# zhangxiaochen95/uav_bs_ctrl

Measured on AMD Instinct MI355X. Metric: env-steps/sec (MADRQN, 8 UBS x 80 GT), higher is better.
Workload: dtype f32

## Files before the change

### include/uavgnn.h

```cpp
#ifndef UAVGNN_H
#define UAVGNN_H

#include <stddef.h>
#include <stdint.h>

#ifdef __cplusplus
extern "C" {
#endif

#define UAVGNN_VERSION 101

#define UAVGNN_EINVAL (-1000)
#define UAVGNN_EUNSUPPORTED (-1001)
#define UAVGNN_EWORKSPACE (-1002)

typedef void* uavgnn_stream_t;

int uavgnn_version(void);

const char* uavgnn_strerror(int code);

int uavgnn_gatv2_fwd(const float* x_src, int E, int F_src, const float* x_dst, int F_dst, const int32_t* seg_off,
                     const int32_t* dst_order, int N, const float* W_s, const float* b_s, const float* W_d, const float* b_d, const float* attn,
                     const float* W_r, const float* b_r, int nh, int D, float slope, float* out, int ld_out,
// ... 205 lines not shown
int uavgnn_gru_cell_x3_supported(int K_in, int H);
long long uavgnn_gru_cell_x3_workspace_bytes(int K_in, int H);
int uavgnn_gru_split_weights(const float* W_ih, int K_in, const float* W_hh, int H, void* planes, uavgnn_stream_t stream);
int uavgnn_gru_cell_fwd_x3(const float* inp, int ld_inp, int K_in, const float* h, int N, int H, const void* planes,
                           const float* b_ih, const float* b_hh, float* h_out, float* pre_save, uavgnn_stream_t stream);
int uavgnn_gru_cell_fwd_x3_cat(const float* inp, int ld_inp, int K1, const float* inp2, int ld_inp2, int K2, const float* h,
                               int N, int H, const void* planes, const float* b_ih, const float* b_hh, float* h_out,
                               float* pre_save, uavgnn_stream_t stream);
#define UAVGNN_GRU_STAGING_BLOCKS 1
int uavgnn_gru_cell_fwd_x3_opts(const float* inp, int ld_inp, int K1, const float* inp2, int ld_inp2, int K2, const float* h,
                                int N, int H, const void* planes, const float* b_ih, const float* b_hh, float* h_out,
                                float* pre_save, int flags, uavgnn_stream_t stream);
int uavgnn_gru_cell_h2_supported(int K_in, int H);
long long uavgnn_gru_cell_h2_workspace_bytes(int K_in, int H);
int uavgnn_gru_split_weights_h2(const float* W_ih, int K_in, const float* W_hh, int H, void* planes, uavgnn_stream_t stream);
int uavgnn_gru_cell_fwd_h2(const float* inp, int ld_inp, int K1, const float* inp2, int ld_inp2, int K2, const float* h, int N, int H,
                           const float* row_absmax, const void* planes, const float* b_ih, const float* b_hh, float* h_out,
                           float* pre_save, uavgnn_stream_t stream);
int uavgnn_row_absmax(const float* a1, int ld1, int K1, const float* a2, int ld2, int K2, const float* a3, int ld3, int K3, int N,
                      float* out, uavgnn_stream_t stream);
int uavgnn_head_supported(int H, int A);
int uavgnn_head_fwd(const float* h, int ld_h, int N, int H, const float* W, int ld_w, const float* b, int A, float* q, int ld_q,
                    uavgnn_stream_t stream);
int uavgnn_head_duel_supported(int H, int A);
int uavgnn_head_fwd_duel(const float* h, int ld_h, int N, int H, const float* W_adv, int ld_w, const float* w_v, const float* b_adv,
                         const float* b_v, int A, float* q, int ld_q, uavgnn_stream_t stream);
int uavgnn_gru_rec_supported(int H);
int uavgnn_gru_rec_fwd(const float* gi, int ld_gi, const float* h, int ld_h, int N, int H, const float* W_hh, const float* b_hh,
                       float* h_out, int ld_ho, float* pre_save, uavgnn_stream_t stream);
int uavgnn_gru_rec_bwd(const float* pre, const float* h, int ld_h, const float* d_hout, const float* d_carry, int N, int H,
                       const float* W_hh, float* d_gi, float* d_gh, float* dh_prev, uavgnn_stream_t stream);
#define UAVGNN_GEMM_ACCUMULATE 1
#define UAVGNN_GEMM_RELU 2
#define UAVGNN_GEMM_STAGING_INTERLEAVED 4
#define UAVGNN_GEMM_TILE_128 8
#define UAVGNN_GEMM_TILE_64 16
int uavgnn_gemm_x3_supported(int M, int N, int K);
int uavgnn_split_bf16x3(const float* W, int ld, int R, int C, int transpose, void* planes, uavgnn_stream_t stream);
int uavgnn_gemm_nt_x3(const float* X, int ldx, int M, int K, const void* planes, int N, const float* bias, float* Y, int ldy,
                      int epilogue, uavgnn_stream_t stream);
int uavgnn_gemm_nt_x3_cat(const float* X, int ldx, int K1, const float* X2, int ldx2, int M, int K, const void* planes, int N,
                          const float* bias, float* Y, int ldy, int epilogue, uavgnn_stream_t stream);
int uavgnn_gemm_nt_x3_rowmax(const float* X, int ldx, int M, int K, const void* planes, int N, const float* bias, float* Y, int ldy,
                             int epilogue, float* rowmax_out, uavgnn_stream_t stream);

int uavgnn_gemm_tn_x3_chunks(long long n_rows, int Mo, int Ko);
int uavgnn_gemm_tn_x3(const float* dY, int ldy, int Mo, const float* X, int ldx, int Ko, long long n_rows, float* partials,
                      int S, int accumulate, uavgnn_stream_t stream);
int uavgnn_col_absmax(const float* x, long long ld, long long n, int C, float* out, uavgnn_stream_t stream);
int uavgnn_gemm_tn_h2_supported(long long n_rows, int Mo, int Ko);
int uavgnn_gemm_tn_h2_chunks(long long n_rows, int Mo, int Ko);
int uavgnn_gemm_tn_h2(const float* dY, long long ldy, int Mo, const float* X, long long ldx, int Ko, long long n_rows,
                      const float* colmax_y, const float* colmax_x, float* partials, int S, int accumulate, uavgnn_stream_t stream);
int uavgnn_gru_gates_bwd_fused(const float* pre, const float* h, const float* d_hout, int N, int H, float* d_gi, float* d_gh,
                               float* d_h, uavgnn_stream_t stream);
int uavgnn_gru_gates_bwd_fused_head(const float* pre, const float* h, const float* d_hout, const float* dq, int n_out,
                                    const float* W_out, int N, int H, float* d_gi, float* d_gh, float* d_h,
                                    uavgnn_stream_t stream);
int uavgnn_gru_gates_bwd_sum_rows(int N, int H);
int uavgnn_gru_gates_bwd_fused_sums(const float* pre, const float* h, const float* d_hout, const float* dq, int n_out,
                                    const float* W_out, int N, int H, float* d_gi, float* d_gh, float* d_h, float* col_sums,
                                    uavgnn_stream_t stream);

long long uavgnn_gru_cell_bwd_workspace_bytes(int K_in, int H);
int uavgnn_gru_split_weights_bwd(const float* W_ih, int K_in, const float* W_hh, int H, void* planes, uavgnn_stream_t stream);
int uavgnn_gru_cell_bwd(const float* pre, const float* h, const float* d_hout, int N, int K_in, int H, const void* planes_bwd,
                        float* d_gi, float* d_gh, float* d_inp, int ld_dinp, float* d_h, uavgnn_stream_t stream);

#define UAVGNN_WS_GATV2_BWD 1
#define UAVGNN_WS_DEGREE_ORDER 2
#define UAVGNN_WS_CSC_TRANSPOSE 3
#define UAVGNN_WS_GRU_PLANES 4
#define UAVGNN_WS_GRU_BWD_PLANES 5
#define UAVGNN_WS_GEMM_PLANES 6
#define UAVGNN_WS_GEMM_TN_PARTIALS 7
#define UAVGNN_WS_K1_IMAGE 8
long long uavgnn_workspace_bytes(int kind, long long a, long long b, long long c);

#ifdef __cplusplus
}
#endif
#endif
```

### uav_bs_ctrl_amd/_lib.py

```python
from __future__ import annotations

import ctypes
import os

import torch as th

_HERE = os.path.dirname(os.path.abspath(__file__))
LIB_PATH = os.environ.get("UAVGNN_LIB") or os.path.join(_HERE, "csrc", "libuavgnn.so")

_c_fp = ctypes.c_void_p
_c_ip = ctypes.c_void_p
_c_int = ctypes.c_int
_c_f32 = ctypes.c_float
_c_st = ctypes.c_void_p

SIGNATURES = {
    "uavgnn_version": (_c_int, []),
    "uavgnn_strerror": (ctypes.c_char_p, [_c_int]),
    "uavgnn_gatv2_fwd": (_c_int, [_c_fp, _c_int, _c_int, _c_fp, _c_int, _c_ip, _c_ip, _c_int, _c_fp, _c_fp, _c_fp, _c_fp, _c_fp,
                                  _c_fp, _c_fp, _c_int, _c_int, _c_f32, _c_fp, _c_int, _c_fp, _c_st]),
    "uavgnn_gatv2_fwd_valu": (_c_int, [_c_fp, _c_int, _c_int, _c_fp, _c_int, _c_ip, _c_ip, _c_int, _c_fp, _c_fp, _c_fp, _c_fp, _c_fp,
                                       _c_fp, _c_fp, _c_int, _c_int, _c_f32, _c_fp, _c_int, _c_fp, _c_st]),
    "uavgnn_gatv2_fwd_mfma": (_c_int, [_c_fp, _c_int, _c_int, _c_fp, _c_int, _c_ip, _c_ip, _c_int, _c_fp, _c_fp, _c_fp, _c_fp, _c_fp,
                                       _c_fp, _c_fp, _c_int, _c_int, _c_f32, _c_fp, _c_int, _c_fp, _c_st]),
# ... 38 lines not shown
    "uavgnn_talk_compact": (_c_int, [_c_fp, _c_int, _c_int, _c_f32, _c_ip, _c_ip, _c_ip, _c_ip, _c_st]),
    "uavgnn_build_graph_small_max_agents": (_c_int, []),
    "uavgnn_build_graph_small": (_c_int, [_c_fp, _c_int, _c_int, _c_fp, _c_int, _c_int, _c_fp, _c_int, _c_int, _c_f32, _c_ip, _c_ip,
                                          _c_ip, _c_fp, _c_fp, _c_ip, _c_ip, _c_ip, _c_st]),
    "uavgnn_degree_order_workspace_bytes": (ctypes.c_size_t, [_c_int]),
    "uavgnn_degree_order": (_c_int, [_c_ip, _c_int, _c_ip, ctypes.c_void_p, ctypes.c_size_t, _c_st]),
    "uavgnn_csc_transpose_workspace_bytes": (ctypes.c_size_t, [_c_int]),
    "uavgnn_csc_transpose": (_c_int, [_c_ip, _c_ip, _c_int, _c_int, _c_ip, _c_ip, _c_ip, ctypes.c_void_p,
                                      ctypes.c_size_t, _c_st]),
    "uavgnn_csc_transpose_env": (_c_int, [_c_ip, _c_ip, _c_ip, _c_int, _c_int, _c_ip, _c_ip, _c_ip, _c_st]),
    "uavgnn_talk_attn_env_supported": (_c_int, [_c_int, _c_int, _c_int]),
    "uavgnn_tarmac_msg_supported": (_c_int, [_c_int, _c_int, _c_int, _c_int]),
    "uavgnn_tarmac_msg_weight_bytes": (ctypes.c_longlong, [_c_int, _c_int, _c_int]),
    "uavgnn_tarmac_msg_prepare": (_c_int, [_c_fp, _c_int, _c_int, _c_int, _c_int, ctypes.c_void_p, _c_st]),
    "uavgnn_tarmac_msg_fwd": (_c_int, [_c_fp, _c_int, _c_fp, _c_int, _c_int, _c_int, _c_int, ctypes.c_void_p, _c_fp, _c_int, _c_int,
                                       _c_ip, _c_ip, _c_f32, _c_fp, _c_int, _c_fp, _c_fp, _c_int, _c_fp, _c_int, _c_st]),
    "uavgnn_talk_attn_env_fwd": (_c_int, [_c_fp, _c_int, _c_fp, _c_int, _c_fp, _c_int, _c_int, _c_int, _c_ip, _c_ip,
                                          _c_ip, _c_int, _c_int, _c_f32, _c_fp, _c_int, _c_fp, _c_fp, _c_int, _c_int,
                                          _c_st]),
    "uavgnn_talk_attn_env_bwd": (_c_int, [_c_fp, _c_int, _c_fp, _c_int, _c_fp, _c_int, _c_int, _c_int, _c_ip, _c_ip,
                                          _c_ip, _c_int, _c_int, _c_f32, _c_fp, _c_fp, _c_int, _c_fp, _c_int, _c_fp,
                                          _c_int, _c_fp, _c_int, _c_st]),
    "uavgnn_eps_greedy": (_c_int, [_c_fp, _c_int, _c_int, _c_int, _c_int, _c_fp, _c_fp, _c_f32, ctypes.c_void_p, _c_st]),
    "uavgnn_eps_greedy_dev": (_c_int, [_c_fp, _c_int, _c_int, _c_int, _c_int, _c_fp, _c_fp, _c_fp, ctypes.c_void_p, _c_st]),
    "uavgnn_eps_schedule": (_c_int, [ctypes.c_void_p, ctypes.c_longlong, ctypes.c_double, ctypes.c_double, ctypes.c_double, _c_fp, _c_st]),
    "uavgnn_eps_greedy_philox": (_c_int, [_c_fp, _c_int, _c_int, _c_int, _c_int, ctypes.c_void_p, _c_fp, _c_f32, ctypes.c_void_p, _c_st]),
    "uavgnn_stats_push": (_c_int, [ctypes.c_void_p, _c_int, _c_int, _c_int, ctypes.c_void_p, _c_st]),
    "uavgnn_film_click_mubs": (_c_int, [_c_int] * 6 + [_c_fp] * 10 + [_c_st]),
    "uavgnn_film_click_subs": (_c_int, [_c_int] * 4 + [ctypes.c_double, _c_int, _c_int] + [_c_fp] * 17 + [_c_st]),
    "uavgnn_replay_commit": (_c_int, [ctypes.POINTER(ctypes.c_longlong), _c_int, _c_int, _c_int, ctypes.c_void_p, _c_st]),
    "uavgnn_replay_sample": (_c_int, [ctypes.c_void_p, ctypes.c_void_p, _c_int, _c_int, ctypes.c_void_p, _c_ip, _c_st]),
    "uavgnn_replay_gather": (_c_int, [ctypes.POINTER(ctypes.c_longlong), _c_int, ctypes.c_void_p, _c_int, _c_st]),
    "uavgnn_colsum_acc": (_c_int, [_c_fp, ctypes.c_longlong, _c_int, _c_int, _c_fp, _c_int, _c_st]),
    "uavgnn_qmix_mix_fwd": (_c_int, [_c_fp, ctypes.c_longlong, _c_fp, _c_fp, _c_fp, _c_int, _c_int, _c_int, _c_fp, _c_st]),
    "uavgnn_qmix_mix_bwd": (_c_int, [_c_fp, ctypes.c_longlong, _c_fp, _c_fp, _c_fp, _c_int, _c_int, _c_int, _c_fp, ctypes.c_longlong, _c_fp,
                                     _c_fp, _c_int, _c_st]),
    "uavgnn_qmix_mix_bwd_partials": (_c_int, [_c_int, _c_int]),
    "uavgnn_relu_bwd_colsum": (_c_int, [_c_fp, ctypes.c_longlong, _c_fp, ctypes.c_longlong, _c_fp, ctypes.c_longlong, _c_int, _c_int, _c_fp,
                               _c_int, _c_st]),
    "uavgnn_relu_bwd_colsum_rowmax": (_c_int, [_c_fp, ctypes.c_longlong, _c_fp, ctypes.c_longlong, _c_fp, ctypes.c_longlong, _c_int, _c_int,
                                               _c_fp, _c_int, _c_fp, _c_st]),
    "uavgnn_flat_obs_supported": (_c_int, [_c_int, _c_int]),
    "uavgnn_flat_obs_fwd": (_c_int, [_c_fp, ctypes.c_longlong, _c_int, _c_fp, ctypes.c_longlong, _c_int, _c_fp, ctypes.c_longlong, _c_int,
                                     _c_int, _c_fp, _c_fp, _c_int, _c_fp, ctypes.c_longlong, _c_st]),
    "uavgnn_flat_obs_wgrad_chunks": (_c_int, [ctypes.c_longlong, _c_int, _c_int]),
    "uavgnn_flat_obs_wgrad": (_c_int, [_c_fp, ctypes.c_longlong, _c_int, _c_fp, ctypes.c_longlong, _c_int, _c_fp, ctypes.c_longlong, _c_int,
                                       _c_fp, ctypes.c_longlong, _c_int, _c_int, _c_fp, _c_int, _c_int, _c_st]),
    "uavgnn_gemm_nt_x3_rowmax": (_c_int, [_c_fp, _c_int, _c_int, _c_int, ctypes.c_void_p, _c_int, _c_fp, _c_fp, _c_int, _c_int, _c_fp, _c_st]),
    "uavgnn_col_absmax": (_c_int, [_c_fp, ctypes.c_longlong, ctypes.c_longlong, _c_int, _c_fp, _c_st]),
    "uavgnn_gemm_tn_h2_supported": (_c_int, [ctypes.c_longlong, _c_int, _c_int]),
    "uavgnn_gemm_tn_h2_chunks": (_c_int, [ctypes.c_longlong, _c_int, _c_int]),
    "uavgnn_gemm_tn_h2": (_c_int, [_c_fp, ctypes.c_longlong, _c_int, _c_fp, ctypes.c_longlong, _c_int, ctypes.c_longlong, _c_fp, _c_fp, _c_fp,
                                   _c_int, _c_int, _c_st]),
    "uavgnn_gemm_h2_supported": (_c_int, [_c_int, _c_int, _c_int]),
    "uavgnn_split_h2_bytes": (ctypes.c_longlong, [_c_int, _c_int]),
    "uavgnn_split_h2": (_c_int, [_c_fp, _c_int, _c_int, _c_int, _c_int, ctypes.c_void_p, _c_st]),
    "uavgnn_gemm_nt_h2": (_c_int, [_c_fp, _c_int, _c_int, _c_fp, _c_int, _c_int, _c_int, _c_fp, _c_fp, ctypes.c_void_p, _c_int, _c_fp, _c_fp,
                                   _c_int, _c_int, _c_st]),
    "uavgnn_gemm_nt_h2_rm2": (_c_int, [_c_fp, _c_int, _c_int, _c_fp, _c_int, _c_int, _c_int, _c_fp, _c_fp, ctypes.c_void_p, _c_int, _c_fp, _c_fp,
                                       _c_int, _c_int, _c_st]),
    "uavgnn_gemm_nt_h2_n64": (_c_int, [_c_fp, _c_int, _c_int, _c_int, _c_fp, ctypes.c_void_p, _c_int, _c_fp, _c_int, _c_st]),
    "uavgnn_env_state_dim": (_c_int, [_c_int, _c_int, _c_int]),
    "uavgnn_env_step": (_c_int, [ctypes.POINTER(ctypes.c_int32), ctypes.POINTER(ctypes.c_double), _c_int] + [_c_fp] * 22 + [_c_st]),
    "uavgnn_map_sample": (_c_int, [ctypes.POINTER(ctypes.c_int32), ctypes.POINTER(ctypes.c_double), _c_int] + [_c_fp] * 6 + [_c_st]),
    "uavgnn_subs_env_step": (_c_int, [ctypes.POINTER(ctypes.c_int32), ctypes.POINTER(ctypes.c_double), _c_int] + [_c_fp] * 16 + [_c_st]),
    "uavgnn_subs_env_sample": (_c_int, [ctypes.POINTER(ctypes.c_int32), ctypes.POINTER(ctypes.c_double), _c_int] + [_c_fp] * 4 + [_c_st]),
    "uavgnn_adamw_polyak": (_c_int, [_c_fp, _c_fp, _c_fp, _c_fp, _c_fp, ctypes.c_longlong, ctypes.c_longlong, _c_fp, ctypes.c_double,
                                     ctypes.c_double, _c_f32, _c_f32, _c_f32, _c_f32, _c_st]),
    "uavgnn_gru_cell_supported": (_c_int, [_c_int, _c_int]),
    "uavgnn_gru_cell_fwd": (_c_int, [_c_fp, _c_int, _c_int, _c_fp, _c_int, _c_int, _c_fp, _c_fp, _c_fp, _c_fp, _c_fp, _c_fp, _c_st]),
    "uavgnn_gru_cell_x3_supported": (_c_int, [_c_int, _c_int]),
    "uavgnn_gru_cell_x3_workspace_bytes": (ctypes.c_longlong, [_c_int, _c_int]),
    "uavgnn_gru_split_weights": (_c_int, [_c_fp, _c_int, _c_fp, _c_int, ctypes.c_void_p, _c_st]),
    "uavgnn_gru_cell_fwd_x3": (_c_int, [_c_fp, _c_int, _c_int, _c_fp, _c_int, _c_int, ctypes.c_void_p, _c_fp, _c_fp, _c_fp, _c_fp, _c_st]),
    "uavgnn_gru_cell_fwd_x3_cat": (_c_int, [_c_fp, _c_int, _c_int, _c_fp, _c_int, _c_int, _c_fp, _c_int, _c_int, ctypes.c_void_p, _c_fp, _c_fp,
                                            _c_fp, _c_fp, _c_st]),
    "uavgnn_gru_cell_fwd_x3_opts": (_c_int, [_c_fp, _c_int, _c_int, _c_fp, _c_int, _c_int, _c_fp, _c_int, _c_int, ctypes.c_void_p, _c_fp, _c_fp,
                                             _c_fp, _c_fp, _c_int, _c_st]),
    "uavgnn_gru_cell_h2_supported": (_c_int, [_c_int, _c_int]),
    "uavgnn_gru_cell_h2_workspace_bytes": (ctypes.c_longlong, [_c_int, _c_int]),
    "uavgnn_gru_split_weights_h2": (_c_int, [_c_fp, _c_int, _c_fp, _c_int, ctypes.c_void_p, _c_st]),
    "uavgnn_gru_cell_fwd_h2": (_c_int, [_c_fp, _c_int, _c_int, _c_fp, _c_int, _c_int, _c_fp, _c_int, _c_int, _c_fp, ctypes.c_void_p, _c_fp,
                                        _c_fp, _c_fp, _c_fp, _c_st]),
    "uavgnn_row_absmax": (_c_int, [_c_fp, _c_int, _c_int, _c_fp, _c_int, _c_int, _c_fp, _c_int, _c_int, _c_int, _c_fp, _c_st]),
    "uavgnn_tarmac_msg_rowmax_supported": (_c_int, [_c_int, _c_int, _c_int, _c_int]),
    "uavgnn_tarmac_msg_fwd_rowmax": (_c_int, [_c_fp, _c_int, _c_fp, _c_int, _c_int, _c_int, _c_int, ctypes.c_void_p, _c_fp, _c_int, _c_int,
                                              _c_ip, _c_ip, _c_f32, _c_fp, _c_int, _c_fp, _c_fp, _c_int, _c_fp, _c_int, _c_fp, _c_st]),
    "uavgnn_gru_cell_bwd_workspace_bytes": (ctypes.c_longlong, [_c_int, _c_int]),
    "uavgnn_gru_split_weights_bwd": (_c_int, [_c_fp, _c_int, _c_fp, _c_int, ctypes.c_void_p, _c_st]),
    "uavgnn_gru_cell_bwd": (_c_int, [_c_fp, _c_fp, _c_fp, _c_int, _c_int, _c_int, ctypes.c_void_p, _c_fp, _c_fp, _c_fp, _c_int, _c_fp,
                                     _c_st]),
    "uavgnn_workspace_bytes": (ctypes.c_longlong, [_c_int, ctypes.c_longlong, ctypes.c_longlong, ctypes.c_longlong]),
    "uavgnn_gemm_tn_x3_chunks": (_c_int, [ctypes.c_longlong, _c_int, _c_int]),
    "uavgnn_gemm_tn_x3": (_c_int, [_c_fp, _c_int, _c_int, _c_fp, _c_int, _c_int, ctypes.c_longlong, _c_fp, _c_int, _c_int, _c_st]),
    "uavgnn_gemm_x3_supported": (_c_int, [_c_int, _c_int, _c_int]),
    "uavgnn_head_supported": (_c_int, [_c_int, _c_int]),
    "uavgnn_head_fwd": (_c_int, [_c_fp, _c_int, _c_int, _c_int, _c_fp, _c_int, _c_fp, _c_int, _c_fp, _c_int, _c_st]),
    "uavgnn_head_duel_supported": (_c_int, [_c_int, _c_int]),
    "uavgnn_head_fwd_duel": (_c_int, [_c_fp, _c_int, _c_int, _c_int, _c_fp, _c_int, _c_fp, _c_fp, _c_fp, _c_int, _c_fp, _c_int, _c_st]),
    "uavgnn_gru_rec_supported": (_c_int, [_c_int]),
    "uavgnn_gru_rec_fwd": (_c_int, [_c_fp, _c_int, _c_fp, _c_int, _c_int, _c_int, _c_fp, _c_fp, _c_fp, _c_int, _c_fp, _c_st]),
    "uavgnn_gru_rec_bwd": (_c_int, [_c_fp, _c_fp, _c_int, _c_fp, _c_fp, _c_int, _c_int, _c_fp, _c_fp, _c_fp, _c_fp, _c_st]),
    "uavgnn_split_bf16x3": (_c_int, [_c_fp, _c_int, _c_int, _c_int, _c_int, ctypes.c_void_p, _c_st]),
    "uavgnn_gemm_nt_x3": (_c_int, [_c_fp, _c_int, _c_int, _c_int, ctypes.c_void_p, _c_int, _c_fp, _c_fp, _c_int, _c_int, _c_st]),
    "uavgnn_gemm_nt_x3_cat": (_c_int, [_c_fp, _c_int, _c_int, _c_fp, _c_int, _c_int, _c_int, ctypes.c_void_p, _c_int, _c_fp, _c_fp, _c_int,
                              _c_int, _c_st]),
# ... 75 lines not shown
```

### uav_bs_ctrl_amd/csrc/gemm_tn_h2.hip

```cpp
#include "common.h"
#include "f16x2.h"

namespace uavgnn {
namespace {

using namespace h2;

typedef short s16x4 __attribute__((ext_vector_type(4)));
typedef short s16x8 __attribute__((ext_vector_type(8)));

constexpr int TI = 256, TJ = 128, BK = 32, NT = 512;
#ifndef GEMM_TN_H2_SUBE
#define GEMM_TN_H2_SUBE 528
#endif
constexpr int SUBE = GEMM_TN_H2_SUBE;
constexpr int PA = (TI / 16) * SUBE, PB = (TJ / 16) * SUBE;
constexpr int BUF = 2 * PA + 2 * PB;

__device__ __forceinline__ f16x8 tr_frag(const unsigned short* p) {
  typedef __attribute__((address_space(3))) s16x4 lds_s16x4;
  const s16x4 lo = __builtin_amdgcn_ds_read_tr16_b64_v4i16((lds_s16x4*)(p));
  const s16x4 hi = __builtin_amdgcn_ds_read_tr16_b64_v4i16((lds_s16x4*)(p + 4 * 16));
  return __builtin_bit_cast(f16x8, s16x8{lo[0], lo[1], lo[2], lo[3], hi[0], hi[1], hi[2], hi[3]});
}
// ... 120 lines not shown
    lstore(0);
    gload(1);
    __syncthreads();
    const bool early = wave < 4;
    Half f0, f1;
    UAVGNN_TNH2_READ(f0, 0, 0)
    for (int t = 0; t < ns; ++t) {
      UAVGNN_TNH2_READ(f1, t & 1, 1)
      if (early) {
        lstore((t + 1) & 1);
        gload(t + 2);
      }
      __builtin_amdgcn_sched_barrier(0);
      UAVGNN_TNH2_MFMA(f0)
      __builtin_amdgcn_sched_barrier(0);
      if (!early) {
        lstore((t + 1) & 1);
        gload(t + 2);
      }
      __syncthreads();
      UAVGNN_TNH2_READ(f0, (t + 1) & 1, 0)
      __builtin_amdgcn_sched_barrier(0);
      UAVGNN_TNH2_MFMA(f1)
      __builtin_amdgcn_sched_barrier(0);
    }
  } else {
    __syncthreads();
  }
#undef UAVGNN_TNH2_MFMA
#undef UAVGNN_TNH2_TERM
#undef UAVGNN_TNH2_READ
  float* __restrict__ Ps = P + static_cast<size_t>(s) * Mo * Ko;
  const int l32 = lane & 31, lh = lane >> 5;
#pragma unroll
  for (int b = 0; b < 2; ++b) {
    const int lcol = 16 * (wcx + 2 * b + 4 * (l32 >> 4)) + (l32 & 15), col = n0 + lcol;
    if (col >= Ko) continue;
    const float cj = sInvB[lcol];
#pragma unroll
    for (int a = 0; a < 2; ++a)
#pragma unroll
      for (int i = 0; i < 16; ++i) {
        const int i32 = 8 * (i >> 2) + 4 * lh + (i & 3);
        const int lrow = 16 * (wr + 8 * a + 4 * (i32 >> 4)) + (i32 & 15), row = m0 + lrow;
        if (row < Mo) {
          float* p = Ps + static_cast<size_t>(row) * Ko + col;
          const float v = acc[a][b][i] * cj * sInvA[lrow];
          *p = ACC ? *p + v : v;
        }
      }
  }
}

}
}

using namespace uavgnn;

extern "C" int uavgnn_col_absmax(const float* x, long long ld, long long n, int C, float* out, uavgnn_stream_t stream) {
  if (!x || !out || n <= 0 || C <= 0 || ld < C) return UAVGNN_EINVAL;
  if ((C & 3) || (ld & 3) || (reinterpret_cast<uintptr_t>(x) & 15)) return UAVGNN_EUNSUPPORTED;
  hipStream_t st = static_cast<hipStream_t>(stream);
  if (hipMemsetAsync(out, 0, sizeof(float) * C, st) != hipSuccess) return launch_status();
  const int gy = (C + 255) / 256;
  long long gx = (n + 63) / 64;
  if (gx > 2048 / gy) gx = 2048 / gy;
  if (gx < 1) gx = 1;
  hipLaunchKernelGGL(col_absmax_kernel, dim3(static_cast<unsigned>(gx), gy), dim3(256), 0, st, x, ld, n, C,
                     reinterpret_cast<unsigned*>(out));
  return launch_status();
}

extern "C" int uavgnn_gemm_tn_h2_supported(long long n_rows, int Mo, int Ko) {
  return (n_rows > 0 && (n_rows % BK) == 0 && Mo >= 4 && Ko >= 4 && (Mo % 4) == 0 && (Ko % 4) == 0) ? 1 : 0;
}

extern "C" int uavgnn_gemm_tn_h2_chunks(long long n_rows, int Mo, int Ko) {
  if (!uavgnn_gemm_tn_h2_supported(n_rows, Mo, Ko)) return 0;
  const int tiles = ((Mo + TI - 1) / TI) * ((Ko + TJ - 1) / TJ);
  long long S = 512 / tiles;
  if (S >= 8) S = S / 8 * 8;
  if (S < 1) S = 1;
  const long long max_s = n_rows / 512 > 0 ? n_rows / 512 : 1;
  if (S > max_s) S = max_s;
  return static_cast<int>(S);
}

extern "C" int uavgnn_gemm_tn_h2(const float* dY, long long ldy, int Mo, const float* X, long long ldx, int Ko, long long n_rows,
                                 const float* colmax_y, const float* colmax_x, float* partials, int S, int accumulate,
                                 uavgnn_stream_t stream) {
  if (!dY || !X || !partials || !colmax_y || !colmax_x || Mo <= 0 || Ko <= 0 || n_rows <= 0 || S <= 0 || ldy < Mo || ldx < Ko)
    return UAVGNN_EINVAL;
  if (!uavgnn_gemm_tn_h2_supported(n_rows, Mo, Ko) || (ldy & 3) || (ldx & 3) || ldy >= (1LL << 31) || ldx >= (1LL << 31) ||
      ((reinterpret_cast<uintptr_t>(dY) | reinterpret_cast<uintptr_t>(X) | reinterpret_cast<uintptr_t>(colmax_y) |
        reinterpret_cast<uintptr_t>(colmax_x)) & 15) || (reinterpret_cast<uintptr_t>(partials) & 3))
    return UAVGNN_EUNSUPPORTED;
  long long chunk = (n_rows + S - 1) / S;
  chunk = (chunk + BK - 1) / BK * BK;
  const int col_blocks = (Ko + TJ - 1) / TJ, row_blocks = (Mo + TI - 1) / TI, tiles = row_blocks * col_blocks;
  const dim3 grid(static_cast<unsigned>(tiles) * S), block(NT);
  hipStream_t st = static_cast<hipStream_t>(stream);
  if (accumulate)
    hipLaunchKernelGGL(gemm_tn_h2_kernel<true>, grid, block, 0, st, dY, static_cast<int>(ldy), Mo, X, static_cast<int>(ldx), Ko, n_rows,
                       chunk, colmax_y, colmax_x, partials, col_blocks, tiles, S);
  else
    hipLaunchKernelGGL(gemm_tn_h2_kernel<false>, grid, block, 0, st, dY, static_cast<int>(ldy), Mo, X, static_cast<int>(ldx), Ko, n_rows,
                       chunk, colmax_y, colmax_x, partials, col_blocks, tiles, S);
  return launch_status();
}
```

### uav_bs_ctrl_amd/ops.py

```python
from __future__ import annotations

import os
import torch as th

from . import _lib as L

NEG_SLOPE = 0.2
K1_IMAGE = os.environ.get("UAVGNN_K1_IMAGE", "1") != "0"
HETERO_FUSED = True
K1_BF16Z = os.environ.get("UAVGNN_K1_BF16Z", "1") != "0"
K1_ROWMAX = os.environ.get("UAVGNN_K1_ROWMAX", "1") != "0"
K1_ROWMAX_MIN_ROWS = 1 << 17
K1_ROWMAX_DENSE_DEG = int(os.environ.get("UAVGNN_K1_ROWMAX_DENSE_DEG", "16"))
K1_ROWMAX_DENSE_MIN_ROWS = 16384


class _KernelTimer:

    def __init__(self):
        self.enabled = False
        self.only = None
        self._spans = {}

    def reset(self, enabled=True, only=None):
# ... 523 lines not shown
        lib, st = L.lib(), L.stream()
        pre_p, h_p, dh_p, gi_p, gh_p, c_p = (t.data_ptr() for t in (pre, hbuf, d_hall, d_gi, d_gh, carry))
        with KERNEL_TIMER.span("gru_rec_bwd", (T1, N, H)):
            for t in range(T1 - 1, -1, -1):
                rc = lib.uavgnn_gru_rec_bwd(pre_p + 16 * t * N * H, h_p + 4 * t * N * H, H, dh_p + 4 * t * N * H,
                                            None if t == T1 - 1 else c_p + 4 * ((t + 1) & 1) * N * H, N, H, W.data_ptr(),
                                            gi_p + 12 * t * N * H, gh_p + 12 * t * N * H, c_p + 4 * (t & 1) * N * H, st)
                L.check(rc, "uavgnn_gru_rec_bwd")
        d_gh2 = d_gh.view(T1 * N, 3 * H)
        dW = _wgrad(d_gh2, hbuf[:T1].view(T1 * N, H)) if ctx.needs_input_grad[2] else None
        db = _colsum(d_gh2) if ctx.needs_input_grad[3] else None
        return d_gi.view(T1 * N, 3 * H), (carry[0] if ctx.needs_input_grad[1] else None), dW, db, None, None


def gru_unroll(x_all, h0, cell, T1):
    N = x_all.shape[0] // T1
    if h0.shape[0] != N:
        h0 = h0.expand(N, -1)
    H = h0.shape[1]
    if not L.lib().uavgnn_gru_rec_supported(H):
        raise L.UavGnnError(f"gru_unroll: no instantiation for H = {H} (uavgnn_gru_rec_supported)")
    gi_all = linear(x_all, cell.weight_ih, cell.bias_ih)
    train = th.is_grad_enabled() and any(t.requires_grad for t in (gi_all, h0, cell.weight_hh, cell.bias_hh))
    return _GruRecurrence.apply(gi_all, h0, cell.weight_hh, cell.bias_hh, T1, train)


def _row_blocks(n, cap=256, min_rows=32):
    S = 1
    while S < cap and n % (2 * S) == 0 and n // (2 * S) >= min_rows:
        S *= 2
    return S


def _colsum_partial(dy):
    n = dy.shape[0]
    S = _row_blocks(n)
    return dy.unflatten(0, (S, n // S)).sum(1)


def _colsum(dy):
    return _colsum_partial(dy).sum(0)


GEMM_X3 = os.environ.get("UAVGNN_GEMM_X3", "1") != "0"


GEMM_X3_FLAGS = {"8": 0, "9": 4, "4": 8}.get(os.environ.get("UAVGNN_GEMM_X3_VARIANT", "8"), 0)
GRU_X3_FLAGS = 1 if os.environ.get("UAVGNN_GRU_X3_VARIANT", "1") == "0" else 0


GEMM_X3_SMALL_GRID = 128


def gemm_x3_supported(a, n_out, k) -> bool:
    return bool(GEMM_X3 and a.is_cuda and a.dtype == th.float32 and a.dim() == 2 and _mc_operand(a) and n_out % 128 == 0 and a.shape[0] >= 4096
                and a.shape[0] * a.stride(0) < 2 ** 31 and L.lib().uavgnn_gemm_x3_supported(a.shape[0], n_out, k))


def gemm_x3(a, W, transpose_w=False, bias=None, out=None, accumulate=False, relu=False, rowmax_out=None):
    lib = L.lib()
    M, K = a.shape
    R, C = W.shape
    n_out = C if transpose_w else R
    assert (R if transpose_w else C) == K and W.stride(1) == 1
    if out is None:
        out = th.empty((M, n_out), dtype=th.float32, device=a.device)
    with KERNEL_TIMER.span("gemm_x3", (M, n_out, K)):
        planes = _weight_planes("mat", (W,), (R, C, int(transpose_w)), 6 * R * C,
                                lambda p: L.check(lib.uavgnn_split_bf16x3(W.data_ptr(), W.stride(0), R, C, int(transpose_w),
                                                                          p.data_ptr(), L.stream()), "uavgnn_split_bf16x3"))
        flags = GEMM_X3_FLAGS
        if not (flags & 8) and ((M + 255) // 256) * ((n_out + 127) // 128) < GEMM_X3_SMALL_GRID:
            flags |= 8
            if ((M + 127) // 128) * ((n_out + 127) // 128) < GEMM_X3_SMALL_GRID:
                flags = (flags & ~8) | 16
        epi = (1 if accumulate else 0) | (2 if relu else 0) | flags
        if rowmax_out is not None and not (flags & 24):
            rc = lib.uavgnn_gemm_nt_x3_rowmax(a.data_ptr(), a.stride(0), M, K, planes.data_ptr(), n_out, L.ptr(bias), out.data_ptr(),
                                              out.stride(0), epi, rowmax_out.data_ptr(), L.stream())
        else:
            if rowmax_out is not None:
                rowmax_out.copy_(a.abs().amax(1))
            rc = lib.uavgnn_gemm_nt_x3(a.data_ptr(), a.stride(0), M, K, planes.data_ptr(), n_out, L.ptr(bias), out.data_ptr(),
                                       out.stride(0), epi, L.stream())
    L.check(rc, "uavgnn_gemm_nt_x3")
    return out


def _mm_nt(x, W, b=None, relu=False):
    if gemm_x3_supported(x, W.shape[0], W.shape[1]) and W.stride(1) == 1 and (b is None or b.is_contiguous()):
        return gemm_x3(x, W, False, bias=b, relu=relu)
    if relu:
        return th._addmm_activation(b, x, W.t())
    return th.addmm(b, x, W.t()) if b is not None else th.mm(x, W.t())


def _mm_nn(dy, W, out=None, accumulate=False, rowmax=None):
    operands_ok = W.stride(1) == 1 and (out is None or (out.stride(1) == 1 and out.dtype == th.float32))
    if rowmax is not None and gemm_h2_supported(dy, W.shape[1], W.shape[0]) and operands_ok:
        return gemm_h2(dy, W, rowmax, True, out=out, accumulate=accumulate)
    if gemm_x3_supported(dy, W.shape[1], W.shape[0]) and operands_ok:
        return gemm_x3(dy, W, True, out=out, accumulate=accumulate)
    if out is None:
        return th.mm(dy, W)
    return out.addmm_(dy, W) if accumulate else th.mm(dy, W, out=out)


def gemm_x3_cat_supported(a1, a2, n_out) -> bool:
# ... 44 lines not shown
            Wc = th.cat((W, W2), 0)
            L.check(lib.uavgnn_split_h2(Wc.data_ptr(), n_out, K, n_out, 1, p.data_ptr(), L.stream()), "uavgnn_split_h2")
    else:
        R, C = W.shape
        n_out, K = (C, R) if transpose_w else (R, C)
        assert K == K1 and W.stride(1) == 1
        tag, weights, dims = "h2mat", (W,), (R, C, int(transpose_w))

        def build(p):
            L.check(lib.uavgnn_split_h2(W.data_ptr(), W.stride(0), R, C, int(transpose_w), p.data_ptr(), L.stream()), "uavgnn_split_h2")
    if out is None:
        out = th.empty((M, n_out), dtype=th.float32, device=a.device)
    with KERNEL_TIMER.span("gemm_h2", (M, n_out, K)):
        planes = _weight_planes(tag, weights, dims, lib.uavgnn_split_h2_bytes(n_out, K), build)
        fn, rm2 = (lib.uavgnn_gemm_nt_h2, rowmax2) if rowmax2_out is None else (lib.uavgnn_gemm_nt_h2_rm2, rowmax2_out)
        rc = fn(a.data_ptr(), a.stride(0), K1, L.ptr(a2), 0 if a2 is None else a2.stride(0), M, K, rowmax.data_ptr(),
                L.ptr(rm2), planes.data_ptr(), n_out, L.ptr(bias), out.data_ptr(), out.stride(0),
                (1 if accumulate else 0) | (2 if relu else 0) | (GEMM_X3_FLAGS & 4), L.stream())
    L.check(rc, "uavgnn_gemm_nt_h2")
    return out


G4 = os.environ.get("UAVGNN_G4", "1") != "0"
DC_H2 = os.environ.get("UAVGNN_DC_H2", "1") != "0"
GEMM_H2_N64_MIN_GRID = 128


def gemm_h2_n64_supported(a, n_out, k) -> bool:
    return bool(DC_H2 and GEMM_H2 and a.is_cuda and a.dtype == th.float32 and a.dim() == 2 and _mc_operand(a) and a.shape[1] == k
                and n_out % 64 == 0 and k % 64 == 0 and a.shape[0] * a.stride(0) < 2 ** 31
                and L.lib().uavgnn_gemm_h2_supported(a.shape[0], n_out, k)
                and ((a.shape[0] + 127) // 128) * (n_out // 64) >= GEMM_H2_N64_MIN_GRID)


def gemm_h2_n64(a, W, rowmax, out=None):
    lib = L.lib()
    M, K = a.shape
    R, n_out = W.shape
    assert R == K and W.stride(1) == 1
    if out is None:
        out = th.empty((M, n_out), dtype=th.float32, device=a.device)
    with KERNEL_TIMER.span("gemm_h2_n64", (M, n_out, K)):
        planes = _weight_planes("h2mat", (W,), (R, n_out, 1), lib.uavgnn_split_h2_bytes(n_out, K),
                                lambda p: L.check(lib.uavgnn_split_h2(W.data_ptr(), W.stride(0), R, n_out, 1, p.data_ptr(), L.stream()),
                                                  "uavgnn_split_h2"))
        rc = lib.uavgnn_gemm_nt_h2_n64(a.data_ptr(), a.stride(0), M, K, rowmax.data_ptr(), planes.data_ptr(), n_out, out.data_ptr(),
                                       out.stride(0), L.stream())
    L.check(rc, "uavgnn_gemm_nt_h2_n64")
    return out


GEMM_TN_MIN_ROWS = 1 << 18
GEMM_TN_H2 = os.environ.get("UAVGNN_GEMM_TN_H2", "1") != "0"


def _max_two_stage(t):
    n = t.numel()
    S = 1
    while S < 1024 and n % (2 * S) == 0 and n // (2 * S) >= 256:
        S *= 2
    return t.reshape(S, n // S).max(1).values.max()


def _gemm_tn_h2_shape(n, Mo, Ko, min_in=128) -> bool:
    return bool(GEMM_X3 and GEMM_H2 and GEMM_TN_H2 and n >= GEMM_TN_MIN_ROWS
                and Mo >= 256 and Ko >= min_in
                and L.lib().uavgnn_gemm_tn_h2_supported(n, Mo, Ko))


def gemm_tn_h2_supported(dy, x, min_in=128) -> bool:
    return bool(dy.is_cuda and dy.dtype == th.float32 and x.dtype == th.float32 and dy.dim() == 2 and x.dim() == 2
                and dy.shape[0] == x.shape[0] and _mc_operand(dy) and _mc_operand(x)
                and _gemm_tn_h2_shape(dy.shape[0], dy.shape[1], x.shape[1], min_in))


def gemm_tn_x3_supported(dy, x) -> bool:
    return bool(GEMM_X3 and dy.is_cuda and dy.dtype == th.float32 and x.dtype == th.float32 and dy.dim() == 2
                and x.dim() == 2 and dy.shape[0] == x.shape[0] and dy.shape[0] >= GEMM_TN_MIN_ROWS and dy.stride(1) == 1
                and x.stride(1) == 1 and dy.shape[1] > 0 and x.shape[1] > 0)


def gemm_tn_x3(dy, x, partials=None, accumulate=False):
    lib = L.lib()
    n, Mo, Ko = dy.shape[0], dy.shape[1], x.shape[1]
    if partials is None:
        S = lib.uavgnn_gemm_tn_x3_chunks(n, Mo, Ko)
        partials = th.empty((S, Mo, Ko), dtype=th.float32, device=dy.device)
    with KERNEL_TIMER.span("gemm_tn_x3", (n, Mo, Ko)):
        rc = lib.uavgnn_gemm_tn_x3(dy.data_ptr(), dy.stride(0), Mo, x.data_ptr(), x.stride(0), Ko, n, partials.data_ptr(),
                                   partials.shape[0], int(accumulate), L.stream())
    L.check(rc, "uavgnn_gemm_tn_x3")
    return partials


def _wgrad_partials(dy, x, bounds=None, allow_tn=True, slot=None):
    n, Mo, Ko = dy.shape[0], dy.shape[1], x.shape[1]
    if bounds is not None:
        tag, S = "tnh2", L.lib().uavgnn_gemm_tn_h2_chunks(n, Mo, Ko)
    elif allow_tn and gemm_tn_x3_supported(dy, x):
        tag, S = "tn", L.lib().uavgnn_gemm_tn_x3_chunks(n, Mo, Ko)
    else:
        tag, S = None, WeightGradSink._chunks(n)
    part, accumulate = slot(tag, (S, Mo, Ko)) if slot is not None else (None, False)
    if part is None and tag is not None:
        part = th.empty((S, Mo, Ko), dtype=th.float32, device=x.device)
    if tag == "tnh2":
        cy, cx = bounds[0].expand(Mo).contiguous(), bounds[1].expand(Ko).contiguous()
        with KERNEL_TIMER.span("gemm_tn_h2", (n, Mo, Ko)):
            rc = L.lib().uavgnn_gemm_tn_h2(dy.data_ptr(), dy.stride(0), Mo, x.data_ptr(), x.stride(0), Ko, n, cy.data_ptr(), cx.data_ptr(),
                                           part.data_ptr(), S, int(accumulate), L.stream())
        L.check(rc, "uavgnn_gemm_tn_h2")
    elif tag == "tn":
        gemm_tn_x3(dy, x, part, accumulate)
    elif S > 1:
        xc = x if x.is_contiguous() else x.contiguous()
        a, b = dy.view(S, n // S, -1).transpose(1, 2), xc.view(S, n // S, -1)
        part = th.bmm(a, b) if part is None else part.baddbmm_(a, b, beta=int(accumulate))
    elif part is None:
        part = th.mm(dy.t(), x).unsqueeze(0)
    else:
        part[0].addmm_(dy.t(), x, beta=int(accumulate))
    return part


def _wgrad(dy, x, bounds=None):
    part = _wgrad_partials(dy, x, bounds)
    return part[0] if part.shape[0] == 1 else part.sum(0)


class _LinearSplitK(th.autograd.Function):

    @staticmethod
    def forward(ctx, x, W, b):
        ctx.save_for_backward(x, W)
        ctx.has_bias = b is not None
        return _mm_nt(x, W, b)

    @staticmethod
    def backward(ctx, dy):
        x, W = ctx.saved_tensors
        return _LinearSplitK._grads(ctx, x, W, dy, ctx.has_bias)

    @staticmethod
    def _grads(ctx, x, W, dy, has_bias, rowmax=None, x_rowmax=None):
        dy = dy.contiguous()
        dx = dW = db = None
        if ctx.needs_input_grad[0]:
            dx = _mm_nn(dy, W, rowmax=rowmax)
        if ctx.needs_input_grad[1]:
            h2 = rowmax is not None and x_rowmax is not None and gemm_tn_h2_supported(dy, x)
            dW = _wgrad(dy, x, (_max_two_stage(rowmax), _max_two_stage(x_rowmax)) if h2 else None)
        if has_bias and ctx.needs_input_grad[2]:
            db = _colsum(dy)
        return dx, dW, db


def linear(x, W, b=None):
    return _LinearSplitK.apply(x, W, b)


QMIX_MAX_AGENTS, QMIX_MAX_EMBED = 16, 128


# ... 813 lines not shown
```

Baseline: 2.721 million.

## Add variable-width column tiles (96/160) to the h2 weight-gradient GEMM

Adds a templated variant of the fp16-split transposed weight-gradient GEMM kernel whose column tile width is 32*M (96 or 160). The width is chosen automatically from Ko's divisibility, so widths that are not multiples of 128 no longer waste padded tile columns. The chunk count is recomputed from the new tile count. It adds more register and LDS pressure for the 160-wide variant, plus wave-role asymmetry between waves that load the middle and last column blocks.

```diff
diff --git a/include/uavgnn.h b/include/uavgnn.h
--- a/include/uavgnn.h
+++ b/include/uavgnn.h
@@ -281,6 +281,11 @@
 int uavgnn_gemm_tn_h2_chunks(long long n_rows, int Mo, int Ko);
 int uavgnn_gemm_tn_h2(const float* dY, long long ldy, int Mo, const float* X, long long ldx, int Ko, long long n_rows,
                       const float* colmax_y, const float* colmax_x, float* partials, int S, int accumulate, uavgnn_stream_t stream);
+int uavgnn_gemm_tn_h2_width(int Ko);
+int uavgnn_gemm_tn_h2_chunks_tj(long long n_rows, int Mo, int Ko, int tj);
+int uavgnn_gemm_tn_h2_tj(const float* dY, long long ldy, int Mo, const float* X, long long ldx, int Ko, long long n_rows,
+                         const float* colmax_y, const float* colmax_x, float* partials, int S, int accumulate, int tj,
+                         uavgnn_stream_t stream);
 int uavgnn_gru_gates_bwd_fused(const float* pre, const float* h, const float* d_hout, int N, int H, float* d_gi, float* d_gh,
                                float* d_h, uavgnn_stream_t stream);
 int uavgnn_gru_gates_bwd_fused_head(const float* pre, const float* h, const float* d_hout, const float* dq, int n_out,
diff --git a/uav_bs_ctrl_amd/_lib.py b/uav_bs_ctrl_amd/_lib.py
--- a/uav_bs_ctrl_amd/_lib.py
+++ b/uav_bs_ctrl_amd/_lib.py
@@ -114,6 +114,10 @@
     "uavgnn_gemm_tn_h2_chunks": (_c_int, [ctypes.c_longlong, _c_int, _c_int]),
     "uavgnn_gemm_tn_h2": (_c_int, [_c_fp, ctypes.c_longlong, _c_int, _c_fp, ctypes.c_longlong, _c_int, ctypes.c_longlong, _c_fp, _c_fp, _c_fp,
                                    _c_int, _c_int, _c_st]),
+    "uavgnn_gemm_tn_h2_width": (_c_int, [_c_int]),
+    "uavgnn_gemm_tn_h2_chunks_tj": (_c_int, [ctypes.c_longlong, _c_int, _c_int, _c_int]),
+    "uavgnn_gemm_tn_h2_tj": (_c_int, [_c_fp, ctypes.c_longlong, _c_int, _c_fp, ctypes.c_longlong, _c_int, ctypes.c_longlong, _c_fp, _c_fp, _c_fp,
+                                      _c_int, _c_int, _c_int, _c_st]),
     "uavgnn_gemm_h2_supported": (_c_int, [_c_int, _c_int, _c_int]),
     "uavgnn_split_h2_bytes": (ctypes.c_longlong, [_c_int, _c_int]),
     "uavgnn_split_h2": (_c_int, [_c_fp, _c_int, _c_int, _c_int, _c_int, ctypes.c_void_p, _c_st]),
diff --git a/uav_bs_ctrl_amd/csrc/gemm_tn_h2.hip b/uav_bs_ctrl_amd/csrc/gemm_tn_h2.hip
--- a/uav_bs_ctrl_amd/csrc/gemm_tn_h2.hip
+++ b/uav_bs_ctrl_amd/csrc/gemm_tn_h2.hip
@@ -196,6 +196,177 @@
   }
 }
 
+template <int M>
+struct TnW {
+  static constexpr int TJW = 32 * M, NQ = M / 2, MT = M - 1;
+  static constexpr int XH = 576, XP = XH + 512;
+  static constexpr int PBW = M * XP;
+  static constexpr int BUFW = 2 * PA + 2 * PBW;
+};
+
+template <int M, bool ACC>
+__global__ __launch_bounds__(NT) void gemm_tn_h2w_kernel(const float* __restrict__ Yd, int ldy, int Mo, const float* __restrict__ X,
+                                                         int ldx, int Ko, long long n_rows, long long chunk,
+                                                         const float* __restrict__ cmax_y, const float* __restrict__ cmax_x,
+                                                         float* __restrict__ P, int col_blocks, int tiles, int S_all) {
+  constexpr int TJW = TnW<M>::TJW, NQ = TnW<M>::NQ, MT = TnW<M>::MT, XH = TnW<M>::XH, XP = TnW<M>::XP, PBW = TnW<M>::PBW, BUFW = TnW<M>::BUFW;
+  __shared__ __attribute__((aligned(16))) unsigned short smem[2 * BUFW];
+  __shared__ float sInvA[TI], sInvB[TJW];
+  const int tid = threadIdx.x, lane = tid & 63, wave = tid >> 6;
+  int tile, s;
+  {
+    const int id = blockIdx.x;
+    if ((S_all & 7) == 0) {
+      const int xcd = id & 7, k = id >> 3;
+      tile = k % tiles;
+      s = (k / tiles) * 8 + xcd;
+    } else {
+      tile = id % tiles;
+      s = id / tiles;
+    }
+  }
+  const int rb = tile / col_blocks, cb = tile - rb * col_blocks;
+  const int m0 = rb * TI, n0 = cb * TJW;
+  const long long r_begin = static_cast<long long>(s) * chunk, r_end = min(r_begin + chunk, n_rows);
+  const int ns = r_begin < r_end ? static_cast<int>((r_end - r_begin) / BK) : 0;
+
+  f32x16 acc[M];
+#pragma unroll
+  for (int b = 0; b < M; ++b)
+#pragma unroll
+    for (int i = 0; i < 16; ++i) acc[b][i] = 0.f;
+
+  const bool last = wave >= 4;
+  const int xr = 4 * (lane >> 5) + ((lane >> 2) & 3), xh = (lane >> 4) & 1, xc = 16 * xh + 4 * (lane & 3);
+  const int bm = wave % MT, gm = (wave / MT) * NQ, gl = wave & 3;
+  const int ca = min(m0 + 4 * (tid & 63), Mo - 4);
+  const int cxm = min(n0 + 32 * bm + xc, Ko - 4), cxl = min(n0 + 32 * MT + xc, Ko - 4);
+  const int ka = tid >> 6;
+  float4 sca, scm, scl;
+  {
+    const float4 ma = *reinterpret_cast<const float4*>(cmax_y + ca), mm = *reinterpret_cast<const float4*>(cmax_x + cxm),
+                 ml = *reinterpret_cast<const float4*>(cmax_x + cxl);
+    sca = make_float4(pow2f(scale_exp(ma.x)), pow2f(scale_exp(ma.y)), pow2f(scale_exp(ma.z)), pow2f(scale_exp(ma.w)));
+    scm = make_float4(pow2f(scale_exp(mm.x)), pow2f(scale_exp(mm.y)), pow2f(scale_exp(mm.z)), pow2f(scale_exp(mm.w)));
+    scl = make_float4(pow2f(scale_exp(ml.x)), pow2f(scale_exp(ml.y)), pow2f(scale_exp(ml.z)), pow2f(scale_exp(ml.w)));
+  }
+  if (tid < TI) sInvA[tid] = pow2f(-scale_exp(cmax_y[min(m0 + tid, Mo - 1)]));
+  if (tid < TJW) sInvB[tid] = pow2f(-scale_exp(cmax_x[min(n0 + tid, Ko - 1)]));
+  const float* pa = Yd + (r_begin + ka) * ldy + ca;
+  const float* pxm = X + (r_begin + 8 * gm + xr) * ldx + cxm;
+  const float* pxl = X + (r_begin + 8 * gl + xr) * ldx + cxl;
+  const long long step_a = 8LL * ldy, step_x = 8LL * ldx;
+  const int wa = ((tid & 63) >> 2) * SUBE + ka * 16 + 4 * (tid & 3);
+  const int xo = xh * XH + xr * 16 + 4 * (lane & 3);
+  const int wxm = bm * XP + xo + 8 * gm * 16, wxl = MT * XP + xo + 8 * gl * 16;
+  float4 ra[4], rxm[NQ], rxl;
+  auto gload = [&](int t) {
+    const long long off = static_cast<long long>(min(t, ns - 1)) * BK;
+#pragma unroll
+    for (int q = 0; q < 4; ++q) ra[q] = *reinterpret_cast<const float4*>(pa + off * ldy + q * step_a);
+#pragma unroll
+    for (int q = 0; q < NQ; ++q) rxm[q] = *reinterpret_cast<const float4*>(pxm + off * ldx + q * step_x);
+    if (last) rxl = *reinterpret_cast<const float4*>(pxl + off * ldx);
+  };
+  auto lstore = [&](int buf) {
+    unsigned short* sb = smem + buf * BUFW;
+#pragma unroll
+    for (int q = 0; q < 4; ++q) stage4(sb + wa + q * 8 * 16, PA, ra[q], sca);
+#pragma unroll
+    for (int q = 0; q < NQ; ++q) stage4(sb + 2 * PA + wxm + q * 8 * 16, PBW, rxm[q], scm);
+    if (last) stage4(sb + 2 * PA + wxl, PBW, rxl, scl);
+  };
+  const int fr = (8 * (lane >> 5) + ((lane & 15) >> 2)) * 16 + 4 * (lane & 3);
+  const int p = (wave & 3) + 8 * (wave >> 2);
+  const int foa = ((lane >> 4) & 1) * 4 * SUBE + fr + p * SUBE, fox = 2 * PA + ((lane >> 4) & 1) * XH + fr;
+  struct Half {
+    f16x8 a[2], b[M][2];
+  };
+#define UAVGNN_TNH2W_READ(F, buf, kh)                                                     \
+  {                                                                                       \
+    const unsigned short* sb = smem + (buf) * BUFW + (kh) * 16 * 16;                      \
+    _Pragma("unroll") for (int pl = 0; pl < 2; ++pl) {                                    \
+      F.a[pl] = tr_frag(sb + foa + pl * PA);                                              \
+      _Pragma("unroll") for (int b = 0; b < M; ++b) F.b[b][pl] = tr_frag(sb + fox + pl * PBW + b * XP); \
+    }                                                                                     \
+  }
+#define UAVGNN_TNH2W_TERM(ia, ib) \
+  _Pragma("unroll") for (int b = 0; b < M; ++b) acc[b] = mfma32(F.a[ia], F.b[b][ib], acc[b]);
+#define UAVGNN_TNH2W_MFMA(F_)                                                  \
+  {                                                                            \
+    const Half& F = F_;                                                        \
+    UAVGNN_TNH2W_TERM(0, 1) UAVGNN_TNH2W_TERM(1, 0) UAVGNN_TNH2W_TERM(0, 0)    \
+  }
+  if (ns > 0) {
+    gload(0);
+    lstore(0);
+    gload(1);
+    __syncthreads();
+    const bool early = wave < 4;
+    Half f0, f1;
+    UAVGNN_TNH2W_READ(f0, 0, 0)
+    for (int t = 0; t < ns; ++t) {
+      UAVGNN_TNH2W_READ(f1, t & 1, 1)
+      if (early) {
+        lstore((t + 1) & 1);
+        gload(t + 2);
+      }
+      __builtin_amdgcn_sched_barrier(0);
+      UAVGNN_TNH2W_MFMA(f0)
+      __builtin_amdgcn_sched_barrier(0);
+      if (!early) {
+        lstore((t + 1) & 1);
+        gload(t + 2);
+      }
+      __syncthreads();
+      UAVGNN_TNH2W_READ(f0, (t + 1) & 1, 0)
+      __builtin_amdgcn_sched_barrier(0);
+      UAVGNN_TNH2W_MFMA(f1)
+      __builtin_amdgcn_sched_barrier(0);
+    }
+  } else {
+    __syncthreads();
+  }
+#undef UAVGNN_TNH2W_MFMA
+#undef UAVGNN_TNH2W_TERM
+#undef UAVGNN_TNH2W_READ
+  float* __restrict__ Ps = P + static_cast<size_t>(s) * Mo * Ko;
+  const int l32 = lane & 31, lh = lane >> 5;
+#pragma unroll
+  for (int b = 0; b < M; ++b) {
+    const int lcol = 32 * b + l32, col = n0 + lcol;
+    if (col >= Ko) continue;
+    const float cj = sInvB[lcol];
+#pragma unroll
+    for (int i = 0; i < 16; ++i) {
+      const int i32 = 8 * (i >> 2) + 4 * lh + (i & 3);
+      const int lrow = 16 * (p + 4 * (i32 >> 4)) + (i32 & 15), row = m0 + lrow;
+      if (row < Mo) {
+        float* q = Ps + static_cast<size_t>(row) * Ko + col;
+        const float v = acc[b][i] * cj * sInvA[lrow];
+        *q = ACC ? *q + v : v;
+      }
+    }
+  }
+}
+
+int tn_width(int Ko) {
+  if (Ko % 128 == 0) return 128;
+  if (Ko % 160 == 0) return 160;
+  if (Ko % 96 == 0) return 96;
+  return 128;
+}
+
+int tn_chunks(long long n_rows, int Mo, int Ko, int tj) {
+  const int tiles = ((Mo + TI - 1) / TI) * ((Ko + tj - 1) / tj);
+  long long S = 512 / tiles;
+  if (S >= 8) S = S / 8 * 8;
+  if (S < 1) S = 1;
+  const long long max_s = n_rows / 512 > 0 ? n_rows / 512 : 1;
+  if (S > max_s) S = max_s;
+  return static_cast<int>(S);
+}
+
 }
 }
 
@@ -219,36 +390,53 @@
   return (n_rows > 0 && (n_rows % BK) == 0 && Mo >= 4 && Ko >= 4 && (Mo % 4) == 0 && (Ko % 4) == 0) ? 1 : 0;
 }
 
-extern "C" int uavgnn_gemm_tn_h2_chunks(long long n_rows, int Mo, int Ko) {
+extern "C" int uavgnn_gemm_tn_h2_width(int Ko) { return Ko > 0 ? tn_width(Ko) : 0; }
+
+extern "C" int uavgnn_gemm_tn_h2_chunks_tj(long long n_rows, int Mo, int Ko, int tj) {
   if (!uavgnn_gemm_tn_h2_supported(n_rows, Mo, Ko)) return 0;
-  const int tiles = ((Mo + TI - 1) / TI) * ((Ko + TJ - 1) / TJ);
-  long long S = 512 / tiles;
-  if (S >= 8) S = S / 8 * 8;
-  if (S < 1) S = 1;
-  const long long max_s = n_rows / 512 > 0 ? n_rows / 512 : 1;
-  if (S > max_s) S = max_s;
-  return static_cast<int>(S);
-}
-
-extern "C" int uavgnn_gemm_tn_h2(const float* dY, long long ldy, int Mo, const float* X, long long ldx, int Ko, long long n_rows,
-                                 const float* colmax_y, const float* colmax_x, float* partials, int S, int accumulate,
-                                 uavgnn_stream_t stream) {
+  if (tj == 0) tj = tn_width(Ko);
+  if (tj != 96 && tj != 128 && tj != 160) return 0;
+  return tn_chunks(n_rows, Mo, Ko, tj);
+}
+
+extern "C" int uavgnn_gemm_tn_h2_chunks(long long n_rows, int Mo, int Ko) { return uavgnn_gemm_tn_h2_chunks_tj(n_rows, Mo, Ko, 0); }
+
+extern "C" int uavgnn_gemm_tn_h2_tj(const float* dY, long long ldy, int Mo, const float* X, long long ldx, int Ko, long long n_rows,
+                                    const float* colmax_y, const float* colmax_x, float* partials, int S, int accumulate, int tj,
+                                    uavgnn_stream_t stream) {
   if (!dY || !X || !partials || !colmax_y || !colmax_x || Mo <= 0 || Ko <= 0 || n_rows <= 0 || S <= 0 || ldy < Mo || ldx < Ko)
     return UAVGNN_EINVAL;
+  if (tj == 0) tj = tn_width(Ko);
+  if (tj != 96 && tj != 128 && tj != 160) return UAVGNN_EINVAL;
   if (!uavgnn_gemm_tn_h2_supported(n_rows, Mo, Ko) || (ldy & 3) || (ldx & 3) || ldy >= (1LL << 31) || ldx >= (1LL << 31) ||
       ((reinterpret_cast<uintptr_t>(dY) | reinterpret_cast<uintptr_t>(X) | reinterpret_cast<uintptr_t>(colmax_y) |
         reinterpret_cast<uintptr_t>(colmax_x)) & 15) || (reinterpret_cast<uintptr_t>(partials) & 3))
     return UAVGNN_EUNSUPPORTED;
   long long chunk = (n_rows + S - 1) / S;
   chunk = (chunk + BK - 1) / BK * BK;
-  const int col_blocks = (Ko + TJ - 1) / TJ, row_blocks = (Mo + TI - 1) / TI, tiles = row_blocks * col_blocks;
+  const int col_blocks = (Ko + tj - 1) / tj, row_blocks = (Mo + TI - 1) / TI, tiles = row_blocks * col_blocks;
+  if (static_cast<long long>(tiles) * S >= (1LL << 31)) return UAVGNN_EUNSUPPORTED;
   const dim3 grid(static_cast<unsigned>(tiles) * S), block(NT);
   hipStream_t st = static_cast<hipStream_t>(stream);
-  if (accumulate)
-    hipLaunchKernelGGL(gemm_tn_h2_kernel<true>, grid, block, 0, st, dY, static_cast<int>(ldy), Mo, X, static_cast<int>(ldx), Ko, n_rows,
-                       chunk, colmax_y, colmax_x, partials, col_blocks, tiles, S);
-  else
-    hipLaunchKernelGGL(gemm_tn_h2_kernel<false>, grid, block, 0, st, dY, static_cast<int>(ldy), Mo, X, static_cast<int>(ldx), Ko, n_rows,
-                       chunk, colmax_y, colmax_x, partials, col_blocks, tiles, S);
+#define UAVGNN_TNH2_LAUNCH(K)                                                                                                         \
+  hipLaunchKernelGGL(K, grid, block, 0, st, dY, static_cast<int>(ldy), Mo, X, static_cast<int>(ldx), Ko, n_rows, chunk, colmax_y, \
+                     colmax_x, partials, col_blocks, tiles, S)
+  if (tj == 128) {
+    if (accumulate) UAVGNN_TNH2_LAUNCH(gemm_tn_h2_kernel<true>);
+    else UAVGNN_TNH2_LAUNCH(gemm_tn_h2_kernel<false>);
+  } else if (tj == 160) {
+    if (accumulate) UAVGNN_TNH2_LAUNCH((gemm_tn_h2w_kernel<5, true>));
+    else UAVGNN_TNH2_LAUNCH((gemm_tn_h2w_kernel<5, false>));
+  } else {
+    if (accumulate) UAVGNN_TNH2_LAUNCH((gemm_tn_h2w_kernel<3, true>));
+    else UAVGNN_TNH2_LAUNCH((gemm_tn_h2w_kernel<3, false>));
+  }
+#undef UAVGNN_TNH2_LAUNCH
   return launch_status();
 }
+
+extern "C" int uavgnn_gemm_tn_h2(const float* dY, long long ldy, int Mo, const float* X, long long ldx, int Ko, long long n_rows,
+                                 const float* colmax_y, const float* colmax_x, float* partials, int S, int accumulate,
+                                 uavgnn_stream_t stream) {
+  return uavgnn_gemm_tn_h2_tj(dY, ldy, Mo, X, ldx, Ko, n_rows, colmax_y, colmax_x, partials, S, accumulate, 0, stream);
+}
diff --git a/uav_bs_ctrl_amd/ops.py b/uav_bs_ctrl_amd/ops.py
--- a/uav_bs_ctrl_amd/ops.py
+++ b/uav_bs_ctrl_amd/ops.py
@@ -599,8 +599,12 @@
 GEMM_X3_SMALL_GRID = 128
 
 
+GEMM_X3_MIN_ROWS = 4096
+
+
 def gemm_x3_supported(a, n_out, k) -> bool:
-    return bool(GEMM_X3 and a.is_cuda and a.dtype == th.float32 and a.dim() == 2 and _mc_operand(a) and n_out % 128 == 0 and a.shape[0] >= 4096
+    return bool(GEMM_X3 and a.is_cuda and a.dtype == th.float32 and a.dim() == 2 and _mc_operand(a) and n_out % 128 == 0
+                and a.shape[0] >= GEMM_X3_MIN_ROWS
                 and a.shape[0] * a.stride(0) < 2 ** 31 and L.lib().uavgnn_gemm_x3_supported(a.shape[0], n_out, k))
 
 
@@ -751,6 +755,7 @@
 
 GEMM_TN_MIN_ROWS = 1 << 18
 GEMM_TN_H2 = os.environ.get("UAVGNN_GEMM_TN_H2", "1") != "0"
+GEMM_TN_TILES = os.environ.get("UAVGNN_GEMM_TN_TILES", "1") != "0"
 
 
 def _max_two_stage(t):
@@ -795,7 +800,8 @@
 def _wgrad_partials(dy, x, bounds=None, allow_tn=True, slot=None):
     n, Mo, Ko = dy.shape[0], dy.shape[1], x.shape[1]
     if bounds is not None:
-        tag, S = "tnh2", L.lib().uavgnn_gemm_tn_h2_chunks(n, Mo, Ko)
+        tag = "tnh2"
+        S = L.lib().uavgnn_gemm_tn_h2_chunks(n, Mo, Ko) if GEMM_TN_TILES else L.lib().uavgnn_gemm_tn_h2_chunks_tj(n, Mo, Ko, 128)
     elif allow_tn and gemm_tn_x3_supported(dy, x):
         tag, S = "tn", L.lib().uavgnn_gemm_tn_x3_chunks(n, Mo, Ko)
     else:
@@ -806,8 +812,10 @@
     if tag == "tnh2":
         cy, cx = bounds[0].expand(Mo).contiguous(), bounds[1].expand(Ko).contiguous()
         with KERNEL_TIMER.span("gemm_tn_h2", (n, Mo, Ko)):
-            rc = L.lib().uavgnn_gemm_tn_h2(dy.data_ptr(), dy.stride(0), Mo, x.data_ptr(), x.stride(0), Ko, n, cy.data_ptr(), cx.data_ptr(),
-                                           part.data_ptr(), S, int(accumulate), L.stream())
+            args = (dy.data_ptr(), dy.stride(0), Mo, x.data_ptr(), x.stride(0), Ko, n, cy.data_ptr(), cx.data_ptr(), part.data_ptr(), S,
+                    int(accumulate))
+            rc = (L.lib().uavgnn_gemm_tn_h2(*args, L.stream()) if GEMM_TN_TILES
+                  else L.lib().uavgnn_gemm_tn_h2_tj(*args, 128, L.stream()))
         L.check(rc, "uavgnn_gemm_tn_h2")
     elif tag == "tn":
         gemm_tn_x3(dy, x, part, accumulate)
```

After: 2.750 million, median of 6. 1.01x the previous value.
